# LepistaBioinformatics/classeq2

Hardware: AMD Instinct MI355X
Metric: query placements/sec, 10k-leaf tree, 150 bp reads (higher is better)
Workload: dtype u64

## Files before the change

### classeq2_amd/csrc/cls_api.cpp

```cpp
#include <hip/hip_runtime.h>
#include <ctype.h>
#include <stdio.h>
#include <stdlib.h>
#include <string.h>

#include <algorithm>
#include <mutex>
#include <new>
#include <string>
#include <thread>
#include <vector>

#include "cls_db.h"
#include "cls_device.h"
#include "cls_extract.h"
#include "cls_kernels.h"
#include "cls_pair.h"
#include "cls_place.h"
#include "cls_tally.h"
#include "cls_tuning.h"

namespace {

thread_local std::string g_err;
// ... 75 lines not shown
    uint64_t ws_seq = 0;
    std::vector<CallSlot> calls;
    struct TreeRow { uint64_t id; uint32_t pre, size; };
    std::vector<TreeRow> tree_rows;
};

namespace cls {
Tuning& tuning() {
    static Tuning t;
    return t;
}
}
namespace {
struct Knob { const char* name; int cls::Tuning::*field; };
const Knob KNOBS[] = {
    {"no_fast", &cls::Tuning::no_fast}, {"no_order", &cls::Tuning::no_order}, {"force_list", &cls::Tuning::force_list},
    {"no_mask_halves", &cls::Tuning::no_mask_halves}, {"no_fat_direct", &cls::Tuning::no_fat_direct}, {"no_tile", &cls::Tuning::no_tile}, {"tile_pass_codes", &cls::Tuning::tile_pass_codes}, {"tile_set_words", &cls::Tuning::tile_set_words}, {"time_class", &cls::Tuning::time_class}, {"tile_one_per_cu", &cls::Tuning::tile_one_per_cu}, {"tile_min_kmers", &cls::Tuning::tile_min_kmers}, {"no_tile_order", &cls::Tuning::no_tile_order}, {"tile_deal", &cls::Tuning::tile_deal}, {"blocks_per_cu", &cls::Tuning::blocks_per_cu}, {"key_blocks_per_cu", &cls::Tuning::key_blocks_per_cu},
    {"long_blocks_per_cu", &cls::Tuning::long_blocks_per_cu}, {"order_mode", &cls::Tuning::order_mode},
    {"order_windows", &cls::Tuning::order_windows}, {"order_both_strands", &cls::Tuning::order_both_strands},
    {"order_block_shift", &cls::Tuning::order_block_shift}, {"order_sample_shift", &cls::Tuning::order_sample_shift},
    {"profile_stop", &cls::Tuning::profile_stop}, {"timing", &cls::Tuning::timing},
    {"build_full_key", &cls::Tuning::build_full_key}, {"tally_no_wave_combine", &cls::Tuning::tally_no_wave_combine},
};
}

extern "C" int cls_set_tuning(const char* name, int value) {
    if (!name) return fail(CLS_E_INVALID_ARG, "cls_set_tuning: null name");
    for (const Knob& k : KNOBS)
        if (strcmp(k.name, name) == 0) { cls::tuning().*(k.field) = value; return CLS_OK; }
    return fail(CLS_E_INVALID_ARG, std::string("cls_set_tuning: unknown knob ") + name);
}
// ... 2078 lines not shown
```

### classeq2_amd/csrc/cls_device.h

```cpp
#pragma once
#include <stdint.h>

#include "cls_place.h"

namespace cls {

struct DNode {
    uint32_t pre;
    uint32_t size;
    uint32_t first_child;
    uint32_t n_nonleaf;
    uint64_t id;
    uint32_t split;
    uint32_t flags;
};
static_assert(sizeof(DNode) == 32, "DNode");

struct Slot {
    uint64_t hash;
    uint64_t loc;
};
static_assert(sizeof(Slot) == 16, "Slot");
constexpr uint64_t SLOT_EMPTY = ~0ULL;
struct TSlot {
// ... 58 lines not shown
    uint32_t max_nonleaf_arity;
    uint32_t format;
    uint32_t addr32;
    uint32_t binary_tree;
    uint32_t canonical;
    uint32_t set_bits;
    uint32_t n_sets;
};

struct PlaceParams {
    int32_t max_iterations;
    uint32_t remove_intersection;
    double min_match_coverage;
};

constexpr uint32_t MAX_READ_KMERS = 64 * 8 * 16;

}
```

### classeq2_amd/csrc/cls_kernels.h

```cpp
#pragma once
#include <hip/hip_runtime.h>

#include <string>
#include <tuple>
#include <type_traits>
#include <utility>

#include "cls_device.h"

namespace cls {

template <int V> using Int = std::integral_constant<int, V>;
template <class F> auto with_bool(bool b, F&& f) { return b ? f(std::true_type{}) : f(std::false_type{}); }
template <class... V> std::string instance_name(const char* kernel, V...) {
    auto arg = [](auto v) { if constexpr (std::is_same_v<decltype(v), bool>) return std::string(v ? "true" : "false"); else return std::to_string(v); };
    std::string s = std::string(kernel) + "<";
    const char* sep = "";
    ((s += sep + arg(V::value), sep = ", "), ...);
    return s + ">";
}
template <class F> struct Pick {
    F* fn;
    size_t smem;
    std::string name;
// ... 23 lines not shown
    uint32_t n_sub;
    TileCfg whole;
    uint64_t scratch_words;
    std::string name;
};

constexpr int N_LISTS = 8;

struct PlacePlan {
    uint32_t grid[2];
    uint32_t grid_blk;
    uint32_t grid_key;
    bool ordered;
    uint64_t keys_off_words;
    uint64_t sort_off_words;
    size_t sort_bytes;
    uint64_t child_off_words;
    uint32_t grid_long;
    uint32_t long_cap;
    uint32_t long_arity;
    uint64_t long_set;
    uint64_t long_stride_words;
    uint64_t long_off_words;
    uint32_t max_kmers;
    bool blk;
    bool tiled;
    TilePlan tile;
    uint32_t tile_from;
    uint64_t tile_off_words;
    enum Timed : uint8_t { TIME_CLASS0, TIME_BLOCK, TIME_TILE } timed;
// ... 18 lines not shown
```

### classeq2_amd/csrc/cls_kernels.hip

```cpp
#include <hip/hip_runtime.h>
#include <stdlib.h>

#include <algorithm>
#include <type_traits>

#include "cls_device.h"
#include "cls_devutil.h"
#include "cls_kernels.h"
#include "cls_murmur.h"
#include "cls_sort.h"
#include "cls_tuning.h"

namespace cls {

namespace {

constexpr int WAVES_PER_BLOCK = 4;
#ifndef MIN_WAVES_PER_EU
#define MIN_WAVES_PER_EU 4
#endif
#ifndef FAST_MIN_WAVES
#define FAST_MIN_WAVES 5
#endif
#ifndef CLS_NARROW_CANON_BITS
// ... 818 lines not shown
    for (int i = 0; i < 4; ++i) r.s[i] = p[i];
    return r;
}

struct FastCtx {
    uint8_t* ascii;
    uint32_t* packed;
    uint32_t* set;
    uint32_t* gkey;
    uint32_t* gcnt;
    uint4* stage;
    uint32_t* ccnt;
    uint32_t* conly;
    uint32_t* cpre;
};
constexpr int FAST_SLOTS_NARROW = 5;
constexpr uint32_t FAST_MAX_ARITY = 256;

struct FatRec { uint32_t x, vlo_lg, vhi_root; };
template <int SET_BITS>
__device__ __forceinline__ void clear_tables(const FastCtx& cx, uint32_t table_bits, uint32_t lane) {
    if constexpr (SET_BITS == 0) {
        if (lane == 0) cx.set[0] = SET_EMPTY;
    } else {
        const uint4 ones = make_uint4(SET_EMPTY, SET_EMPTY, SET_EMPTY, SET_EMPTY), zero = make_uint4(0, 0, 0, 0);
        uint4* const s4 = reinterpret_cast<uint4*>(cx.set);
        uint4* const k4 = reinterpret_cast<uint4*>(cx.gkey);
        uint4* const c4 = reinterpret_cast<uint4*>(cx.gcnt);
#pragma unroll 1
        for (uint32_t i = lane; i < (1u << table_bits) / 4; i += 64) { s4[i] = ones; k4[i] = ones; c4[i] = zero; }
    }
}

template <int SLOTS, int SET_BITS, bool ADDR32, bool FAT = false>
__device__ __forceinline__ bool fast_front(const DbDev& db, const FastCtx& cx, const uint8_t* __restrict__ bases, uint64_t b0,
                                           uint32_t L, uint32_t nf, uint32_t nk, uint32_t (&e)[SLOTS], uint32_t (&key)[SLOTS], uint32_t (&kw)[SLOTS],
                                           FatRec (&rec)[SLOTS], uint32_t sample_shift = 32, bool canonical = false, uint32_t table_bits = SET_BITS) {
    const uint32_t lane = threadIdx.x & 63;
    const uint32_t k = db.k;
    bool bad = false;
#pragma unroll 1
    for (uint32_t i = lane; i < L; i += 64) {
        uint8_t c = bases[b0 + i];
        if (c >= 'a' && c <= 'z') c -= 32;
        bad |= !(c == 'A' || c == 'C' || c == 'G' || c == 'T');
        cx.ascii[i] = c;
    }
    clear_tables<SET_BITS>(cx, table_bits, lane);
    if (__ballot(bad)) return false;
    wave_sync();
    {
        const uint32_t n_words = (L + 15) >> 4;
#pragma unroll 1
        for (uint32_t w = lane; w < n_words; w += 64) {
            uint32_t acc = 0;
#pragma unroll
            for (int q = 0; q < 4; ++q) {
                uint32_t t = *reinterpret_cast<const uint32_t*>(cx.ascii + 16 * w + 4 * q);
                t = (t >> 1) & 0x03030303u;
                t = (t | (t >> 6) | (t >> 12) | (t >> 18)) & 0xFFu;
                acc |= t << (8 * q);
            }
            cx.packed[w] = acc;
        }
    }
    wave_sync();
    const uint32_t* __restrict__ direct = db.direct;
    const uint32_t kmask = (k == 16) ? 0xFFFFFFFFu : ((1u << (2 * k)) - 1u);
#pragma unroll
    for (int s = 0; s < SLOTS; ++s) {
        const uint32_t j = s * 64 + lane;
        const bool valid = j < nk;
        const bool rc = j >= nf;
        const uint32_t p = valid ? (rc ? (nf - 1) - (j - nf) : j) : 0;
        const uint32_t w = p >> 4, sh = (2 * p) & 31;
        const uint32_t d0 = cx.packed[w], d1 = cx.packed[w + 1];
        uint32_t code = (uint32_t)((((uint64_t)d1 << 32) | d0) >> sh) & kmask;
        uint32_t rcc = __builtin_bitreverse32(code ^ (0xAAAAAAAAu & kmask));
        rcc = ((rcc >> 1) & 0x55555555u) | ((rcc & 0x55555555u) << 1);
        rcc >>= (32 - 2 * k);
        const bool palindrome = code == rcc;
        code = canonical ? (rcc < code ? rcc : code) : (rc ? rcc : code);
        const bool take = valid && (sample_shift >= 32 || ((code * 0x9E3779B1u) >> sample_shift) == 0);
        if constexpr (FAT) {
            const uint4 v = ldx<uint4, ADDR32>(reinterpret_cast<const uint4*>(db.direct16), take ? code : 0u);
            e[s] = take ? v.w : 0u;
            rec[s] = FatRec{v.x, take ? v.y : 0xFFFFFFFFu, take ? v.z : 0u};
        } else {
            const uint32_t v = ldx<uint32_t, ADDR32>(direct, take ? code : 0u);
            e[s] = take ? v : 0u;
        }
        key[s] = code;
        kw[s] = !take ? 0u : (canonical && !palindrome) ? 2u : 1u;
    }
    return true;
}

template <int SLOTS, int SET_BITS, bool ADDR32>
__device__ __forceinline__ bool hash_front(const DbDev& db, const FastCtx& cx, const uint8_t* __restrict__ bases, uint64_t b0,
                                           uint32_t L, uint32_t nf, uint32_t nk, uint32_t (&e)[SLOTS], uint32_t (&key)[SLOTS], uint32_t (&kw)[SLOTS],
                                           uint32_t table_bits, uint32_t& ib) {
    const uint32_t lane = threadIdx.x & 63;
    const uint32_t k = db.k, m_eff = db.m_eff;
    bool bad = false;
#pragma unroll 1
    for (uint32_t i = lane; i < L; i += 64) {
        uint8_t c = bases[b0 + i];
        if (c >= 'a' && c <= 'z') c -= 32;
        bad |= !(c == 'A' || c == 'C' || c == 'G' || c == 'T');
// ... 347 lines not shown
            for (uint32_t c = CL; c < n_loop; ++c) {
                uint4 g = cx.stage[c * 64 + lane];
                uint32_t sm, rm_, km;
                classify(g.x, g.y, g.w, sm, rm_, km);
                const uint2 t = request(g.z, rm_);
                finish(g.x, g.y, g.z, g.w, sm, rm_, km, t);
                cx.stage[c * 64 + lane] = g;
            }
        };
        if (right) narrow_side(std::true_type{}); else narrow_side(std::false_type{});
    }
}

template <int SLOTS, int SET_BITS, bool STATS, bool ADDR32, int MODE, bool POLY>
__device__ __forceinline__ void place_read_fast(const DbDev& db, const PlaceParams& prm, const FastCtx& cx,
                                                const uint8_t* __restrict__ bases, uint64_t b0, uint64_t b1, uint32_t r,
                                                cls_placement* __restrict__ out, cls_query_stats* __restrict__ stats,
                                                uint32_t profile_stop_arg) {
#ifdef CLS_PROFILE_HOOKS
    const uint32_t profile_stop = profile_stop_arg;
#else
    constexpr uint32_t profile_stop = 0;
    (void)profile_stop_arg;
#endif
    const uint32_t lane = threadIdx.x & 63;
    const uint32_t k = db.k;
    const uint64_t L64 = b1 - b0;
    auto put_stats = [&](uint32_t nk_, uint32_t nm, uint32_t nr, uint64_t lp) {
        if (STATS && stats && lane == 0) {
            uint64_t* s = reinterpret_cast<uint64_t*>(stats + r);
            s[0] = (uint64_t)nk_ | ((uint64_t)nm << 32);
            s[1] = (uint64_t)nr;
            s[2] = lp;
        }
    };
    if (L64 < k) { put_stats(0, 0, 0, 0); write_record(out, r, CLS_ERR_TOO_FEW_KMERS, 0, 0, 0, 0); return; }
    const uint32_t L = (uint32_t)L64, nf = L - k + 1, nk = 2 * nf;
    constexpr bool CANON = MODE == 1 || MODE == 4, HASHED = MODE == 2, FAT = MODE >= 3;
    constexpr int LS = CANON ? (SLOTS + 1) / 2 : SLOTS;
    uint32_t sid[LS], key[LS], kw[LS];
    FatRec frec[LS];
    uint32_t tb = SET_BITS;
    if constexpr (SET_BITS > 9) {
        const uint32_t want = 2 * (CANON ? nf : nk);
        tb = 9;
        while ((1u << tb) < want && tb < (uint32_t)SET_BITS) ++tb;
        tb = uniform(tb);
    }
    bool valid_read;
    uint32_t ib = 0;
    if constexpr (HASHED) valid_read = hash_front<LS, SET_BITS, ADDR32>(db, cx, bases, b0, L, nf, nk, sid, key, kw, tb, ib);
    else {
        valid_read = fast_front<LS, SET_BITS, ADDR32, FAT>(db, cx, bases, b0, L, nf, CANON ? nf : nk, sid, key, kw, frec, 32, CANON, tb);
        if (STATS) for (int s = 0; s < LS; ++s) ib += kw[s] ? (FAT ? 16u : 4u) : 0u;
    }
    auto put_index_bytes = [&]() {
        if constexpr (STATS) {
            const uint32_t total = wave_sum(ib);
            if (stats && lane == 0) reinterpret_cast<uint32_t*>(stats + r)[3] = total;
        }
    };
    if (!valid_read) {
        put_stats(0, 0, 0, 0);
        write_record(out, r, CLS_ERR_INVALID_BASE, 0, 0, 0, 0);
        return;
    }
    uint32_t nm_lane = 0;
#pragma unroll
    for (int s = 0; s < LS; ++s) {
        sid[s] &= SET_ID_MASK;
        if (sid[s] != 0) {
            uint32_t pos = (key[s] * 2654435761u) >> (32 - tb);
#pragma unroll 1
            for (;;) {
                const uint32_t old = atomicCAS(&cx.set[pos], SET_EMPTY, key[s]);
                if (old == SET_EMPTY) break;
                if (old == key[s]) { sid[s] = 0; kw[s] = 0; break; }
                pos = (pos + 1) & ((1u << tb) - 1);
            }
        }
        nm_lane += sid[s] != 0 ? kw[s] : 0u;
// ... 74 lines not shown
        const uint64_t exp_usize = (expected != expected) ? 0ull : (uint64_t)expected;
        if ((uint64_t)n_root < exp_usize) { put_index_bytes(); write_record(out, r, CLS_UNCLASSIFIABLE_COVERAGE, (int32_t)n_root, 0, 0, 0); return; }
    }
    bool in_registers = false;
    if constexpr (!POLY) in_registers = uniform(n_sets) <= 128;
    constexpr bool REG2 = !POLY || MODE != 2;
    if (in_registers) descend_groups<ADDR32, POLY, STATS, false, REG2>(db, prm, cx, n_sets, P, r, out, ib);
    else descend_groups<ADDR32, POLY, STATS, true, REG2>(db, prm, cx, n_sets, P, r, out, ib);
    put_index_bytes();
}

template <int SLOTS, int SET_BITS, bool STATS, bool ADDR32, int MODE, bool POLY>
__global__ __launch_bounds__(64 * WAVES_PER_BLOCK, SLOTS > 5 ? FAST_MIN_WAVES_WIDE : POLY ? FAST_MIN_WAVES_POLY : FAST_MIN_WAVES) void place_fast_kernel(
    DbDev db, PlaceParams prm, const uint8_t* __restrict__ bases, const uint64_t* __restrict__ offsets,
    const uint32_t* __restrict__ list, const uint32_t* __restrict__ list_len, uint32_t list_n, uint32_t xcd_chunks,
    cls_placement* __restrict__ out, cls_query_stats* __restrict__ stats, uint32_t ascii_cap, uint32_t profile_stop) {
    extern __shared__ __align__(16) uint8_t smem[];
    const uint32_t wave = threadIdx.x >> 6;
    const uint32_t packed_words = MODE == 2 ? 0u : ((ascii_cap >> 4) + 2 + 3) & ~3u;
    constexpr bool FITS = (12u << SET_BITS) >= 16u * 64 * ((MODE == 1 || MODE == 4) ? (SLOTS + 1) / 2 : SLOTS);
    if constexpr (FITS) {
    const uint32_t per_wave = ascii_cap + 4u * packed_words + (12u << SET_BITS) + (POLY ? 12u * FAST_MAX_ARITY + 16u : 0u);
    FastCtx cx;
    cx.ascii = smem + wave * per_wave;
    cx.packed = reinterpret_cast<uint32_t*>(cx.ascii + ascii_cap);
    cx.set = cx.packed + packed_words;
    cx.gkey = cx.set + (1u << SET_BITS);
    cx.gcnt = cx.gkey + (1u << SET_BITS);
    cx.stage = reinterpret_cast<uint4*>(cx.set);
    cx.ccnt = cx.gcnt + (1u << SET_BITS);
    cx.conly = cx.ccnt + FAST_MAX_ARITY;
    cx.cpre = cx.conly + FAST_MAX_ARITY;
    if (xcd_chunks && SLOTS > FAST_SLOTS_NARROW && *list_len == 0) return;
    const uint32_t n_list = xcd_chunks ? list_n : *list_len;
    const uint32_t xcd = blockIdx.x & 7u, bpx = gridDim.x >> 3;
    const uint32_t chunk = xcd_chunks ? (n_list + 7u) >> 3 : n_list;
    const uint32_t first = xcd_chunks ? (blockIdx.x >> 3) * WAVES_PER_BLOCK + wave : blockIdx.x * WAVES_PER_BLOCK + wave;
    const uint32_t stride = (xcd_chunks ? bpx : gridDim.x) * WAVES_PER_BLOCK;
    const uint32_t origin = xcd_chunks ? xcd * chunk : 0u;
    constexpr uint32_t cap = 64 * SLOTS;
    for (uint32_t ql = first; ql < chunk; ql += stride) {
        const uint32_t q = origin + ql;
        if (q >= n_list) break;
        const uint32_t r = list[q];
        const uint64_t b0 = offsets[r], b1 = offsets[r + 1];
        if (xcd_chunks) {
            const uint64_t L64 = b1 - b0;
            if (L64 >= db.k && 2 * (L64 - db.k + 1) > cap) continue;
            if (SLOTS > FAST_SLOTS_NARROW && (L64 < db.k || 2 * (L64 - db.k + 1) <= 64 * FAST_SLOTS_NARROW)) continue;
        }
        place_read_fast<SLOTS, SET_BITS, STATS, ADDR32, MODE, POLY>(db, prm, cx, bases, b0, b1, r, out, stats, profile_stop);
        wave_sync();
    }
    }
}

__device__ __forceinline__ uint64_t make_order_key(uint32_t key_mode, uint32_t median, uint32_t mh_spec, uint32_t mh_all, uint32_t block_shift, uint32_t set_bits) {
    if (key_mode == 1) return ((uint64_t)(mh_all >> 12) << set_bits) | median;
    return ((uint64_t)(median >> block_shift) << 16) | (mh_spec >> 16);
}

template <int SLOTS, bool ADDR32, bool FWD, bool HASHED>
__global__ __launch_bounds__(64 * WAVES_PER_BLOCK) void order_key_kernel(DbDev db, const uint8_t* __restrict__ bases,
                                                                       const uint64_t* __restrict__ offsets, uint32_t n_reads,
                                                                       uint64_t* __restrict__ keys, uint32_t* __restrict__ idx,
                                                                       uint32_t ascii_cap, uint32_t key_mode,
// ... 59 lines not shown
                    }
                    key = make_order_key(key_mode, prefix, mh, mha, block_shift, db.set_bits);
                }
            }
            wave_sync();
        }
        if (lane == 0) { keys[r] = key; idx[r] = r; }
    }
}

template <bool ADDR32>
__global__ __launch_bounds__(64 * WAVES_PER_BLOCK) void order_key_half_kernel(DbDev db, const uint8_t* __restrict__ bases,
                                                                            const uint64_t* __restrict__ offsets, uint32_t n_reads,
                                                                            uint64_t* __restrict__ keys, uint32_t* __restrict__ idx,
                                                                            uint32_t key_mode, uint32_t block_shift,
                                                                            uint32_t key_cap) {
    constexpr uint32_t MAXL = 64 + DIRECT_MAX_K - 1 + 1;
    constexpr uint32_t WORDS = (MAXL + 15) / 16 + 2;
    __shared__ __align__(16) uint8_t s_ascii[WAVES_PER_BLOCK * 2][(MAXL + 19) & ~3u];
    __shared__ uint32_t s_packed[WAVES_PER_BLOCK * 2][WORDS];
    const uint32_t wave = threadIdx.x >> 6, lane = threadIdx.x & 63, half = lane >> 5, hl = lane & 31;
    uint8_t* ascii = s_ascii[wave * 2 + half];
    uint32_t* packed = s_packed[wave * 2 + half];
    const uint32_t k = db.k;
    const uint32_t kmask = (1u << (2 * k)) - 1u;
    const uint32_t* __restrict__ direct = db.direct;
    const uint32_t pair0 = (blockIdx.x * WAVES_PER_BLOCK + wave) * 2, stride = gridDim.x * WAVES_PER_BLOCK * 2;
    auto half_of = [&](uint64_t m) { return (uint32_t)(m >> (32 * half)); };
    for (uint32_t r0 = pair0; r0 < n_reads; r0 += stride) {
        const uint32_t r = r0 + half;
        const bool have = r < n_reads;
        const uint64_t b0 = have ? offsets[r] : 0, L64 = have ? offsets[r + 1] - b0 : 0;
        const bool keyed = have && L64 >= k && 2 * (L64 - k + 1) <= (uint64_t)key_cap;
        const uint32_t L = keyed ? (uint32_t)std::min<uint64_t>(L64, 64 + k - 1) : 0, nf = keyed ? L - k + 1 : 0;
        bool bad = false;
        for (uint32_t i = hl; i < L; i += 32) {
            uint8_t c = bases[b0 + i];
            if (c >= 'a' && c <= 'z') c -= 32;
            bad |= !(c == 'A' || c == 'C' || c == 'G' || c == 'T');
            ascii[i] = c;
        }
        const bool ok = keyed && half_of(__ballot(bad)) == 0;
        wave_sync();
        for (uint32_t w = hl; w < (L + 15) / 16 + 1; w += 32) {
            uint32_t acc = 0;
#pragma unroll
            for (int q = 0; q < 4; ++q) {
                uint32_t t = *reinterpret_cast<const uint32_t*>(ascii + 16 * w + 4 * q);
                t = (t >> 1) & 0x03030303u;
                t = (t | (t >> 6) | (t >> 12) | (t >> 18)) & 0xFFu;
                acc |= t << (8 * q);
            }
            if (w < WORDS) packed[w] = acc;
        }
        wave_sync();
        uint32_t e[2], hs[2];
#pragma unroll
        for (int s = 0; s < 2; ++s) {
            const uint32_t p = hl + 32 * s;
            const bool valid = ok && p < nf;
            const uint32_t w = valid ? p >> 4 : 0, sh = valid ? (2 * p) & 31 : 0;
            const uint32_t d0 = packed[w], d1 = packed[w + 1];
            uint32_t code = (uint32_t)((((uint64_t)d1 << 32) | d0) >> sh) & kmask;
            uint32_t rcc = __builtin_bitreverse32(code ^ (0xAAAAAAAAu & kmask));
            rcc = ((rcc >> 1) & 0x55555555u) | ((rcc & 0x55555555u) << 1);
            rcc >>= (32 - 2 * k);
            code = rcc < code ? rcc : code;
            const uint32_t v = ldx<uint32_t, ADDR32>(direct, valid ? code : 0u);
            e[s] = valid ? v : 0u;
            hs[s] = mix32(code);
// ... 559 lines not shown
}
auto long_kernel(const DbDev& db, bool stats) {
    auto inst = [&](auto... v) { return pick(place_long_kernel<decltype(v)::value...>, 0, "place_long_kernel", v...); };
    return with_bool(db.format == FMT_SPLIT, [&](auto sp) { return with_bool(stats, [&](auto st) { return inst(sp, st); }); });
}

using KeyFn = decltype(order_key_kernel<2, true, true, false>);
using KeyHalfFn = decltype(order_key_half_kernel<true>);
struct KeyKernel {
    KeyFn* full;
    KeyHalfFn* half;
    size_t smem;
    std::string name;
    const void* fn() const { return full ? (const void*)full : (const void*)half; }
};
KeyKernel key_kernel(const DbDev& db, bool sizing) {
    const Tuning& tn = tuning();
    const bool fwd = !tn.order_both_strands, hashed = fast_mode(db) == 2;
    if (!sizing && !hashed && fwd && tn.order_windows == 64 && (uint32_t)tn.order_sample_shift >= 32)
        return with_bool(db.addr32, [&](auto a32) { return KeyKernel{nullptr, order_key_half_kernel<decltype(a32)::value>, 0, instance_name("order_key_half_kernel", a32)}; });
    const uint32_t ac = ascii_cap_of(db, 0);
    const size_t smem = (size_t)WAVES_PER_BLOCK * (ac + (db.direct ? 4u * (((ac >> 4) + 2 + 3) & ~3u) : 0u) + 16u);
    auto inst = [&](auto... v) { return KeyKernel{order_key_kernel<decltype(v)::value...>, nullptr, smem, instance_name("order_key_kernel", v...)}; };
    auto of = [&](auto a32, auto hs) {
        if (fwd && tn.order_windows <= 64) return inst(Int<2>{}, a32, std::true_type{}, hs);
        if (fwd || sizing) return inst(Int<CLS_SLOTS[0]>{}, a32, std::true_type{}, hs);
        return inst(Int<CLS_SLOTS[0]>{}, a32, std::false_type{}, hs);
    };
    if (hashed) return of(std::true_type{}, std::true_type{});
    return db.addr32 ? of(std::true_type{}, std::false_type{}) : of(std::false_type{}, std::false_type{});
}
}

void PlacePlan::class_caps(uint32_t (&cap)[N_LISTS]) const {
// ... 44 lines not shown
        p.grid[0] = std::max<uint32_t>(8, p.grid[0] & ~7u);
        p.grid[1] = std::max<uint32_t>(8, p.grid[1] & ~7u);
        {
            int per_cu = tuning().key_blocks_per_cu;
            const KeyKernel k = key_kernel(db, true);
            if (per_cu <= 0 && (hipOccupancyMaxActiveBlocksPerMultiprocessor(&per_cu, k.fn(), 64 * WAVES_PER_BLOCK, k.smem) != hipSuccess || per_cu <= 0)) per_cu = 4;
            if (tuning().key_blocks_per_cu <= 0 && fast_mode(db) == 2) per_cu *= 2;
            p.grid_key = std::max<uint32_t>(1, std::min<uint32_t>(want, n_cu * (uint32_t)per_cu));
        }
        p.keys_off_words = w;
        w += 6 * (uint64_t)n_reads;
        p.sort_off_words = w;
        p.sort_bytes = order_temp_bytes(n_reads);
        w += (p.sort_bytes + 3) / 4 + 2;
        w += w & 1;
    }
    p.child_off_words = w;
    w += child_words;
    w += w & 1;
    p.max_kmers = n_long ? std::max<uint32_t>(long_cap, 2u) : MAX_READ_KMERS;
    const uint32_t blk_cap = (uint32_t)(64 * BLK_WAVES * BLK_SLOTS);
    p.tile_from = blk_cap;
    if (tile_usable(db)) {
        p.tile_from = tuning().tile_min_kmers > 0 ? std::min<uint32_t>(blk_cap, (uint32_t)tuning().tile_min_kmers) : (uint32_t)(64 * CLS_SLOTS[1]);
        if (p.max_kmers > p.tile_from) {
            p.tile = tile_plan(db, stats, p.tile_from, p.max_kmers, n_reads, n_cu);
            p.tiled = p.tile.whole.cap_kmers > p.tile_from;
        }
    }
    if (p.tiled) {
// ... 32 lines not shown
    for (int c = 0; c < N_LISTS; ++c) lists[c] = d_ws + 16 + (size_t)c * n_reads;
    uint32_t* child_ws = (child_ws_stride(db) && !child_in_lds(db)) ? d_ws + plan.child_off_words : nullptr;
    hipError_t e = hipMemsetAsync(counts, 0, 64, stream);
    if (e != hipSuccess) return e;
    const uint32_t profile_stop = (uint32_t)tuning().profile_stop;
    const uint32_t ws_stride = child_ws_stride(db);
    const bool st = d_stats != nullptr;
    auto classify = [&](const uint32_t* order) {
        ClassCaps caps{};
        plan.class_caps(caps.cap);
        return launch_kernel(classify_kernel, dim3((n_reads + CLASSIFY_THREADS * CLASSIFY_PER_THREAD - 1) / (CLASSIFY_THREADS * CLASSIFY_PER_THREAD)), dim3(CLASSIFY_THREADS), 0,
                             stream, d_offsets, order, n_reads, db.k, caps, lists[0], counts, d_out, d_stats);
    };
    const uint32_t* list0 = lists[0];
    uint32_t list0_n = 0, xcd_chunks = 0;
    if (!plan.ordered) e = classify(nullptr);
    else {
        uint64_t* keys_in = reinterpret_cast<uint64_t*>(d_ws + plan.keys_off_words);
        uint64_t* keys_out = keys_in + n_reads;
        uint32_t* idx_in = reinterpret_cast<uint32_t*>(keys_out + n_reads);
        uint32_t* idx_out = idx_in + n_reads;
        const Tuning& tn = tuning();
        const uint32_t key_mode = (uint32_t)tn.order_mode;
        const uint32_t block_shift = (uint32_t)tn.order_block_shift;
        const uint32_t key_cap = (plan.tiled && !tn.no_tile_order) ? 0xFFFFFFFFu : (uint32_t)(64 * CLS_SLOTS[1]);
        const KeyKernel k = key_kernel(db, false);
        const dim3 block(64 * WAVES_PER_BLOCK);
        if (k.half) {
            const uint32_t grid_half = std::max<uint32_t>(1, std::min<uint32_t>((n_reads + 2 * WAVES_PER_BLOCK - 1) / (2 * WAVES_PER_BLOCK), plan.grid_key));
            e = launch_kernel(k.half, dim3(grid_half), block, k.smem, stream, db, d_bases, d_offsets, n_reads, keys_in, idx_in, key_mode, block_shift, key_cap);
        } else {
            e = launch_kernel(k.full, dim3(plan.grid_key), block, k.smem, stream, db, d_bases, d_offsets, n_reads, keys_in, idx_in, ascii_cap_of(db, 0), key_mode,
                              block_shift, (uint32_t)tn.order_sample_shift, tn.order_both_strands ? 0u : 1u, key_cap);
        }
        if (e != hipSuccess) return e;
        e = order_reads(d_ws + plan.sort_off_words, keys_in, idx_out, n_reads, order_key_bits(db) - 1, stream);
        if (e != hipSuccess) return e;
        list0 = idx_out;
        list0_n = n_reads;
        xcd_chunks = 1;
        e = classify(idx_out);
    }
    if (e != hipSuccess) return e;
    auto launch_class = [&](int c) {
        const ClassKernel k = class_kernel(db, c, st);
        const dim3 grid(plan.grid[c]), block(64 * WAVES_PER_BLOCK);
        if (k.fast) {
            return launch_kernel(k.fast, grid, block, k.smem, stream, db, prm, d_bases, d_offsets, xcd_chunks ? list0 : lists[c], counts + c, list0_n, xcd_chunks,
                                 d_out, d_stats, ascii_cap_of(db, c), profile_stop);
        }
        if (k.split)
            return launch_kernel(k.split, grid, block, k.smem, stream, db, prm, d_bases, d_offsets, lists[c], counts + c, d_out, d_stats, seq_cap_of(db, c),
                                 profile_stop, child_ws, ws_stride);
        return launch_kernel(k.wave, grid, block, k.smem, stream, db, prm, d_bases, d_offsets, lists[c], counts + c, d_out, d_stats, seq_cap_of(db, c), child_ws,
                             ws_stride);
    };
    auto timed = [&](PlacePlan::Timed t, auto&& launch) {
        if (ev_start && plan.timed == t) (void)hipEventRecord(ev_start, stream);
        const hipError_t r = launch();
        if (ev_stop && plan.timed == t) (void)hipEventRecord(ev_stop, stream);
        return r;
    };
    e = timed(PlacePlan::TIME_CLASS0, [&] { return launch_class(0); });
    if (e != hipSuccess) return e;
// ... 31 lines not shown
```

### classeq2_amd/csrc/cls_sort.h

```cpp
#pragma once
#include <hip/hip_runtime.h>
#include <stddef.h>
#include <stdint.h>

namespace cls {
constexpr int ORDER_BIN_BITS = 12;
constexpr uint32_t ORDER_BINS = 1u << ORDER_BIN_BITS;
size_t order_temp_bytes(uint32_t n);
hipError_t order_reads(void* tmp, const uint64_t* keys, uint32_t* idx_out, uint32_t n, int key_bits, hipStream_t stream);
}
```

### classeq2_amd/csrc/cls_sort.hip

```cpp
#include "cls_sort.h"

namespace cls {

namespace {

constexpr int SORT_THREADS = 1024, SORT_PER_THREAD = 16;

__device__ __forceinline__ uint32_t bin_of(uint64_t key, int shift) {
    return key == ~0ull ? ORDER_BINS - 1 : (uint32_t)(key >> shift) & (ORDER_BINS - 1);
}

__global__ __launch_bounds__(SORT_THREADS) void order_hist_kernel(const uint64_t* __restrict__ keys, uint32_t n, int shift, uint32_t* __restrict__ hist,
                                                                 uint32_t* __restrict__ block_base) {
    __shared__ uint32_t h[ORDER_BINS];
    for (uint32_t i = threadIdx.x; i < ORDER_BINS; i += SORT_THREADS) h[i] = 0;
    __syncthreads();
    const uint32_t base = blockIdx.x * (SORT_THREADS * SORT_PER_THREAD);
#pragma unroll
    for (int q = 0; q < SORT_PER_THREAD; ++q) {
        const uint32_t r = base + q * SORT_THREADS + threadIdx.x;
        if (r < n) atomicAdd(&h[bin_of(keys[r], shift)], 1u);
    }
    __syncthreads();
    for (uint32_t i = threadIdx.x; i < ORDER_BINS; i += SORT_THREADS)
// ... 8 lines not shown
    for (uint32_t q = 0; q < PER; ++q) { v[q] = hist[threadIdx.x * PER + q]; sum += v[q]; }
    const uint32_t lane = threadIdx.x & 63, wave = threadIdx.x >> 6;
    uint32_t inc = sum;
#pragma unroll
    for (int o = 1; o < 64; o <<= 1) { const uint32_t t = __shfl_up(inc, o); if ((int)lane >= o) inc += t; }
    if (lane == 63) wave_tot[wave] = inc;
    __syncthreads();
    uint32_t before = 0;
    for (uint32_t w = 0; w < wave; ++w) before += wave_tot[w];
    uint32_t at = before + inc - sum;
#pragma unroll
    for (uint32_t q = 0; q < PER; ++q) { hist[threadIdx.x * PER + q] = at; at += v[q]; }
}

__global__ __launch_bounds__(SORT_THREADS) void order_scatter_kernel(const uint64_t* __restrict__ keys, uint32_t n, int shift, const uint32_t* __restrict__ start,
                                                                    const uint32_t* __restrict__ block_base, uint32_t* __restrict__ idx_out) {
    __shared__ uint32_t at[ORDER_BINS];
    for (uint32_t i = threadIdx.x; i < ORDER_BINS; i += SORT_THREADS) at[i] = start[i] + block_base[(size_t)blockIdx.x * ORDER_BINS + i];
    __syncthreads();
    const uint32_t base = blockIdx.x * (SORT_THREADS * SORT_PER_THREAD);
#pragma unroll
    for (int q = 0; q < SORT_PER_THREAD; ++q) {
        const uint32_t r = base + q * SORT_THREADS + threadIdx.x;
        if (r < n) idx_out[atomicAdd(&at[bin_of(keys[r], shift)], 1u)] = r;
    }
}

}

static uint32_t order_blocks(uint32_t n) { return (n + SORT_THREADS * SORT_PER_THREAD - 1) / (SORT_THREADS * SORT_PER_THREAD); }

size_t order_temp_bytes(uint32_t n) { return (1 + (size_t)order_blocks(n)) * ORDER_BINS * sizeof(uint32_t); }

hipError_t order_reads(void* tmp, const uint64_t* keys, uint32_t* idx_out, uint32_t n, int key_bits, hipStream_t stream) {
    uint32_t* hist = static_cast<uint32_t*>(tmp);
    uint32_t* block_base = hist + ORDER_BINS;
    const int shift = key_bits > ORDER_BIN_BITS ? key_bits - ORDER_BIN_BITS : 0;
    hipError_t e = hipMemsetAsync(hist, 0, ORDER_BINS * sizeof(uint32_t), stream);
    if (e != hipSuccess) return e;
    const uint32_t blocks = order_blocks(n);
    hipLaunchKernelGGL(order_hist_kernel, dim3(blocks), dim3(SORT_THREADS), 0, stream, keys, n, shift, hist, block_base);
    hipLaunchKernelGGL(order_scan_kernel, dim3(1), dim3(1024), 0, stream, hist);
    hipLaunchKernelGGL(order_scatter_kernel, dim3(blocks), dim3(SORT_THREADS), 0, stream, keys, n, shift, (const uint32_t*)hist, (const uint32_t*)block_base, idx_out);
    return hipGetLastError();
}

}
```

### classeq2_amd/csrc/cls_tuning.h

```cpp
#pragma once

namespace cls {

struct Tuning {
    int no_fast = 0;
    int no_order = 0;
    int force_list = 0;
    int no_mask_halves = 0;
    int no_fat_direct = 0;
    int no_tile = 0;
    int tile_pass_codes = 0;
    int tile_set_words = 0;
    int tile_min_kmers = 0;
    int tile_deal = 64;
    int no_tile_order = 0;
    int tile_one_per_cu = 0;
    int time_class = 0;
    int blocks_per_cu = 0;
    int key_blocks_per_cu = 0;
    int long_blocks_per_cu = 2;
    int order_mode = 0;
    int order_windows = 64;
    int order_both_strands = 0;
    int order_block_shift = 2;
// ... 11 lines not shown
```

Measured before the change: 158.0 million.

## Pack narrow reads into 2-bit records in key kernel and scatter them sorted

The order-key kernel, which already reads and validates every base, now also writes a fixed 64-byte record per read holding the read id, length/status header and 2-bit packed bases. The sort scatter step permutes these records into sorted order alongside the index. The narrow fast placement kernel then loads one contiguous record per read instead of gathering ASCII bases through offsets and re-packing them. This removes scattered base gathers and the per-read packing stage from the placement kernel, at the cost of extra workspace and record traffic in the key and scatter kernels.

```diff
diff --git a/classeq2_amd/csrc/cls_api.cpp b/classeq2_amd/csrc/cls_api.cpp
--- a/classeq2_amd/csrc/cls_api.cpp
+++ b/classeq2_amd/csrc/cls_api.cpp
@@ -113,7 +113,7 @@
 namespace {
 struct Knob { const char* name; int cls::Tuning::*field; };
 const Knob KNOBS[] = {
-    {"no_fast", &cls::Tuning::no_fast}, {"no_order", &cls::Tuning::no_order}, {"force_list", &cls::Tuning::force_list},
+    {"no_fast", &cls::Tuning::no_fast}, {"no_order", &cls::Tuning::no_order}, {"no_packed_reads", &cls::Tuning::no_packed_reads}, {"force_list", &cls::Tuning::force_list},
     {"no_mask_halves", &cls::Tuning::no_mask_halves}, {"no_fat_direct", &cls::Tuning::no_fat_direct}, {"no_tile", &cls::Tuning::no_tile}, {"tile_pass_codes", &cls::Tuning::tile_pass_codes}, {"tile_set_words", &cls::Tuning::tile_set_words}, {"time_class", &cls::Tuning::time_class}, {"tile_one_per_cu", &cls::Tuning::tile_one_per_cu}, {"tile_min_kmers", &cls::Tuning::tile_min_kmers}, {"no_tile_order", &cls::Tuning::no_tile_order}, {"tile_deal", &cls::Tuning::tile_deal}, {"blocks_per_cu", &cls::Tuning::blocks_per_cu}, {"key_blocks_per_cu", &cls::Tuning::key_blocks_per_cu},
     {"long_blocks_per_cu", &cls::Tuning::long_blocks_per_cu}, {"order_mode", &cls::Tuning::order_mode},
     {"order_windows", &cls::Tuning::order_windows}, {"order_both_strands", &cls::Tuning::order_both_strands},
diff --git a/classeq2_amd/csrc/cls_device.h b/classeq2_amd/csrc/cls_device.h
--- a/classeq2_amd/csrc/cls_device.h
+++ b/classeq2_amd/csrc/cls_device.h
@@ -96,6 +96,12 @@
     double min_match_coverage;
 };
 
+constexpr uint32_t PACKED_READ_DWORDS = 16, PACKED_READ_WORDS = 12, PACKED_READ_MAX_BASES = 176;
+constexpr uint32_t PACKED_READ_LEN_MASK = 0xFFFFu;
+constexpr uint32_t PACKED_READ_PACKED = 1u << 16;
+constexpr uint32_t PACKED_READ_BAD_BASE = 1u << 17;
+constexpr uint32_t PACKED_READ_OTHER_CLASS = 1u << 18;
+
 constexpr uint32_t MAX_READ_KMERS = 64 * 8 * 16;
 
 }
diff --git a/classeq2_amd/csrc/cls_kernels.h b/classeq2_amd/csrc/cls_kernels.h
--- a/classeq2_amd/csrc/cls_kernels.h
+++ b/classeq2_amd/csrc/cls_kernels.h
@@ -61,6 +61,9 @@
     bool ordered;
     uint64_t keys_off_words;
     uint64_t sort_off_words;
+    bool packed;
+    uint64_t rec_in_off_words;
+    uint64_t rec_sorted_off_words;
     size_t sort_bytes;
     uint64_t child_off_words;
     uint32_t grid_long;
diff --git a/classeq2_amd/csrc/cls_kernels.hip b/classeq2_amd/csrc/cls_kernels.hip
--- a/classeq2_amd/csrc/cls_kernels.hip
+++ b/classeq2_amd/csrc/cls_kernels.hip
@@ -856,6 +856,7 @@
     uint32_t* conly;
     uint32_t* cpre;
 };
+constexpr uint32_t REC_PRESENT = 1u << 31;
 constexpr int FAST_SLOTS_NARROW = 5;
 constexpr uint32_t FAST_MAX_ARITY = 256;
 
@@ -874,12 +875,9 @@
     }
 }
 
-template <int SLOTS, int SET_BITS, bool ADDR32, bool FAT = false>
-__device__ __forceinline__ bool fast_front(const DbDev& db, const FastCtx& cx, const uint8_t* __restrict__ bases, uint64_t b0,
-                                           uint32_t L, uint32_t nf, uint32_t nk, uint32_t (&e)[SLOTS], uint32_t (&key)[SLOTS], uint32_t (&kw)[SLOTS],
-                                           FatRec (&rec)[SLOTS], uint32_t sample_shift = 32, bool canonical = false, uint32_t table_bits = SET_BITS) {
+template <int SET_BITS>
+__device__ __forceinline__ bool fast_stage(const FastCtx& cx, const uint8_t* __restrict__ bases, uint64_t b0, uint32_t L, uint32_t table_bits) {
     const uint32_t lane = threadIdx.x & 63;
-    const uint32_t k = db.k;
     bool bad = false;
 #pragma unroll 1
     for (uint32_t i = lane; i < L; i += 64) {
@@ -906,7 +904,14 @@
             cx.packed[w] = acc;
         }
     }
-    wave_sync();
+    return true;
+}
+
+template <int SLOTS, bool ADDR32, bool FAT>
+__device__ __forceinline__ void fast_lookup(const DbDev& db, const FastCtx& cx, uint32_t nf, uint32_t nk, uint32_t (&e)[SLOTS], uint32_t (&key)[SLOTS],
+                                            uint32_t (&kw)[SLOTS], FatRec (&rec)[SLOTS], uint32_t sample_shift, bool canonical) {
+    const uint32_t lane = threadIdx.x & 63;
+    const uint32_t k = db.k;
     const uint32_t* __restrict__ direct = db.direct;
     const uint32_t kmask = (k == 16) ? 0xFFFFFFFFu : ((1u << (2 * k)) - 1u);
 #pragma unroll
@@ -935,6 +940,15 @@
         key[s] = code;
         kw[s] = !take ? 0u : (canonical && !palindrome) ? 2u : 1u;
     }
+}
+
+template <int SLOTS, int SET_BITS, bool ADDR32, bool FAT = false>
+__device__ __forceinline__ bool fast_front(const DbDev& db, const FastCtx& cx, const uint8_t* __restrict__ bases, uint64_t b0,
+                                           uint32_t L, uint32_t nf, uint32_t nk, uint32_t (&e)[SLOTS], uint32_t (&key)[SLOTS], uint32_t (&kw)[SLOTS],
+                                           FatRec (&rec)[SLOTS], uint32_t sample_shift = 32, bool canonical = false, uint32_t table_bits = SET_BITS) {
+    if (!fast_stage<SET_BITS>(cx, bases, b0, L, table_bits)) return false;
+    wave_sync();
+    fast_lookup<SLOTS, ADDR32, FAT>(db, cx, nf, nk, e, key, kw, rec, sample_shift, canonical);
     return true;
 }
 
@@ -1312,9 +1326,9 @@
 
 template <int SLOTS, int SET_BITS, bool STATS, bool ADDR32, int MODE, bool POLY>
 __device__ __forceinline__ void place_read_fast(const DbDev& db, const PlaceParams& prm, const FastCtx& cx,
-                                                const uint8_t* __restrict__ bases, uint64_t b0, uint64_t b1, uint32_t r,
+                                                const uint8_t* __restrict__ bases, uint64_t b0, uint32_t L, uint32_t r,
                                                 cls_placement* __restrict__ out, cls_query_stats* __restrict__ stats,
-                                                uint32_t profile_stop_arg) {
+                                                uint32_t profile_stop_arg, uint32_t rec_hdr) {
 #ifdef CLS_PROFILE_HOOKS
     const uint32_t profile_stop = profile_stop_arg;
 #else
@@ -1323,7 +1337,6 @@
 #endif
     const uint32_t lane = threadIdx.x & 63;
     const uint32_t k = db.k;
-    const uint64_t L64 = b1 - b0;
     auto put_stats = [&](uint32_t nk_, uint32_t nm, uint32_t nr, uint64_t lp) {
         if (STATS && stats && lane == 0) {
             uint64_t* s = reinterpret_cast<uint64_t*>(stats + r);
@@ -1332,8 +1345,8 @@
             s[2] = lp;
         }
     };
-    if (L64 < k) { put_stats(0, 0, 0, 0); write_record(out, r, CLS_ERR_TOO_FEW_KMERS, 0, 0, 0, 0); return; }
-    const uint32_t L = (uint32_t)L64, nf = L - k + 1, nk = 2 * nf;
+    if (L < k) { put_stats(0, 0, 0, 0); write_record(out, r, CLS_ERR_TOO_FEW_KMERS, 0, 0, 0, 0); return; }
+    const uint32_t nf = L - k + 1, nk = 2 * nf;
     constexpr bool CANON = MODE == 1 || MODE == 4, HASHED = MODE == 2, FAT = MODE >= 3;
     constexpr int LS = CANON ? (SLOTS + 1) / 2 : SLOTS;
     uint32_t sid[LS], key[LS], kw[LS];
@@ -1345,11 +1358,21 @@
         while ((1u << tb) < want && tb < (uint32_t)SET_BITS) ++tb;
         tb = uniform(tb);
     }
+    uint32_t ib = 0;
     bool valid_read;
-    uint32_t ib = 0;
     if constexpr (HASHED) valid_read = hash_front<LS, SET_BITS, ADDR32>(db, cx, bases, b0, L, nf, nk, sid, key, kw, tb, ib);
-    else {
-        valid_read = fast_front<LS, SET_BITS, ADDR32, FAT>(db, cx, bases, b0, L, nf, CANON ? nf : nk, sid, key, kw, frec, 32, CANON, tb);
+    else if (rec_hdr) {
+        valid_read = (rec_hdr & PACKED_READ_PACKED) != 0;
+        if (valid_read) clear_tables<SET_BITS>(cx, tb, lane);
+    } else valid_read = fast_stage<SET_BITS>(cx, bases, b0, L, tb);
+    if (!valid_read) {
+        put_stats(0, 0, 0, 0);
+        write_record(out, r, CLS_ERR_INVALID_BASE, 0, 0, 0, 0);
+        return;
+    }
+    if constexpr (!HASHED) {
+        wave_sync();
+        fast_lookup<LS, ADDR32, FAT>(db, cx, nf, CANON ? nf : nk, sid, key, kw, frec, 32, CANON);
         if (STATS) for (int s = 0; s < LS; ++s) ib += kw[s] ? (FAT ? 16u : 4u) : 0u;
     }
     auto put_index_bytes = [&]() {
@@ -1358,11 +1381,6 @@
             if (stats && lane == 0) reinterpret_cast<uint32_t*>(stats + r)[3] = total;
         }
     };
-    if (!valid_read) {
-        put_stats(0, 0, 0, 0);
-        write_record(out, r, CLS_ERR_INVALID_BASE, 0, 0, 0, 0);
-        return;
-    }
     uint32_t nm_lane = 0;
 #pragma unroll
     for (int s = 0; s < LS; ++s) {
@@ -1467,7 +1485,8 @@
 __global__ __launch_bounds__(64 * WAVES_PER_BLOCK, SLOTS > 5 ? FAST_MIN_WAVES_WIDE : POLY ? FAST_MIN_WAVES_POLY : FAST_MIN_WAVES) void place_fast_kernel(
     DbDev db, PlaceParams prm, const uint8_t* __restrict__ bases, const uint64_t* __restrict__ offsets,
     const uint32_t* __restrict__ list, const uint32_t* __restrict__ list_len, uint32_t list_n, uint32_t xcd_chunks,
-    cls_placement* __restrict__ out, cls_query_stats* __restrict__ stats, uint32_t ascii_cap, uint32_t profile_stop) {
+    cls_placement* __restrict__ out, cls_query_stats* __restrict__ stats, uint32_t ascii_cap, uint32_t profile_stop,
+    const uint32_t* __restrict__ recs) {
     extern __shared__ __align__(16) uint8_t smem[];
     const uint32_t wave = threadIdx.x >> 6;
     const uint32_t packed_words = MODE == 2 ? 0u : ((ascii_cap >> 4) + 2 + 3) & ~3u;
@@ -1495,14 +1514,29 @@
     for (uint32_t ql = first; ql < chunk; ql += stride) {
         const uint32_t q = origin + ql;
         if (q >= n_list) break;
-        const uint32_t r = list[q];
-        const uint64_t b0 = offsets[r], b1 = offsets[r + 1];
-        if (xcd_chunks) {
-            const uint64_t L64 = b1 - b0;
-            if (L64 >= db.k && 2 * (L64 - db.k + 1) > cap) continue;
-            if (SLOTS > FAST_SLOTS_NARROW && (L64 < db.k || 2 * (L64 - db.k + 1) <= 64 * FAST_SLOTS_NARROW)) continue;
-        }
-        place_read_fast<SLOTS, SET_BITS, STATS, ADDR32, MODE, POLY>(db, prm, cx, bases, b0, b1, r, out, stats, profile_stop);
+        uint32_t r, L, rec_hdr = 0;
+        uint64_t b0 = 0;
+        if (SLOTS == FAST_SLOTS_NARROW && MODE != 2 && xcd_chunks && recs) {
+            uint32_t lane = threadIdx.x & 63;
+            asm volatile("" : "+v"(lane));
+            const uint32_t w = lane < PACKED_READ_DWORDS ? recs[(size_t)q * PACKED_READ_DWORDS + lane] : 0u;
+            r = (uint32_t)__builtin_amdgcn_readlane((int)w, 0);
+            rec_hdr = (uint32_t)__builtin_amdgcn_readlane((int)w, 1);
+            if (rec_hdr & PACKED_READ_OTHER_CLASS) continue;
+            if (lane >= 2 && lane < 2 + PACKED_READ_WORDS) cx.packed[lane - 2] = w;
+            L = rec_hdr & PACKED_READ_LEN_MASK;
+            rec_hdr |= REC_PRESENT;
+        } else {
+            r = list[q];
+            b0 = offsets[r];
+            const uint64_t L64 = offsets[r + 1] - b0;
+            if (xcd_chunks) {
+                if (L64 >= db.k && 2 * (L64 - db.k + 1) > cap) continue;
+                if (SLOTS > FAST_SLOTS_NARROW && (L64 < db.k || 2 * (L64 - db.k + 1) <= 64 * FAST_SLOTS_NARROW)) continue;
+            }
+            L = (uint32_t)L64;
+        }
+        place_read_fast<SLOTS, SET_BITS, STATS, ADDR32, MODE, POLY>(db, prm, cx, bases, b0, L, r, out, stats, profile_stop, rec_hdr);
         wave_sync();
     }
     }
@@ -1592,16 +1626,18 @@
                                                                             const uint64_t* __restrict__ offsets, uint32_t n_reads,
                                                                             uint64_t* __restrict__ keys, uint32_t* __restrict__ idx,
                                                                             uint32_t key_mode, uint32_t block_shift,
-                                                                            uint32_t key_cap) {
-    constexpr uint32_t MAXL = 64 + DIRECT_MAX_K - 1 + 1;
-    constexpr uint32_t WORDS = (MAXL + 15) / 16 + 2;
-    __shared__ __align__(16) uint8_t s_ascii[WAVES_PER_BLOCK * 2][(MAXL + 19) & ~3u];
+                                                                            uint32_t key_cap, uint32_t* __restrict__ recs) {
+    constexpr uint32_t MAXL = PACKED_READ_MAX_BASES;
+    constexpr uint32_t WORDS = MAXL / 16 + 2;
+    static_assert(MAXL % 16 == 0 && MAXL >= 64 * FAST_SLOTS_NARROW / 2 + DIRECT_MAX_K - 1 && MAXL / 16 + 1 <= PACKED_READ_WORDS, "packed-read record");
+    __shared__ __align__(16) uint8_t s_ascii[WAVES_PER_BLOCK * 2][MAXL + 16];
     __shared__ uint32_t s_packed[WAVES_PER_BLOCK * 2][WORDS];
     const uint32_t wave = threadIdx.x >> 6, lane = threadIdx.x & 63, half = lane >> 5, hl = lane & 31;
     uint8_t* ascii = s_ascii[wave * 2 + half];
     uint32_t* packed = s_packed[wave * 2 + half];
     const uint32_t k = db.k;
     const uint32_t kmask = (1u << (2 * k)) - 1u;
+    const uint32_t key_len = 64 + k - 1;
     const uint32_t* __restrict__ direct = db.direct;
     const uint32_t pair0 = (blockIdx.x * WAVES_PER_BLOCK + wave) * 2, stride = gridDim.x * WAVES_PER_BLOCK * 2;
     auto half_of = [&](uint64_t m) { return (uint32_t)(m >> (32 * half)); };
@@ -1610,15 +1646,20 @@
         const bool have = r < n_reads;
         const uint64_t b0 = have ? offsets[r] : 0, L64 = have ? offsets[r + 1] - b0 : 0;
         const bool keyed = have && L64 >= k && 2 * (L64 - k + 1) <= (uint64_t)key_cap;
-        const uint32_t L = keyed ? (uint32_t)std::min<uint64_t>(L64, 64 + k - 1) : 0, nf = keyed ? L - k + 1 : 0;
-        bool bad = false;
+        const bool narrow = recs && have && L64 >= k && 2 * (L64 - k + 1) <= (uint64_t)(64 * FAST_SLOTS_NARROW);
+        const uint32_t L = narrow ? (uint32_t)L64 : keyed ? (uint32_t)std::min<uint64_t>(L64, key_len) : 0;
+        const uint32_t nf = keyed ? std::min<uint32_t>(L, key_len) - k + 1 : 0;
+        bool bad = false, bad_key = false;
         for (uint32_t i = hl; i < L; i += 32) {
             uint8_t c = bases[b0 + i];
             if (c >= 'a' && c <= 'z') c -= 32;
-            bad |= !(c == 'A' || c == 'C' || c == 'G' || c == 'T');
+            const bool b = !(c == 'A' || c == 'C' || c == 'G' || c == 'T');
+            bad |= b;
+            bad_key |= b && i < key_len;
             ascii[i] = c;
         }
-        const bool ok = keyed && half_of(__ballot(bad)) == 0;
+        const bool ok = keyed && half_of(__ballot(bad_key)) == 0;
+        const bool all_ok = half_of(__ballot(bad)) == 0;
         wave_sync();
         for (uint32_t w = hl; w < (L + 15) / 16 + 1; w += 32) {
             uint32_t acc = 0;
@@ -1629,9 +1670,18 @@
                 t = (t | (t >> 6) | (t >> 12) | (t >> 18)) & 0xFFu;
                 acc |= t << (8 * q);
             }
+            const uint32_t in = 16 * w >= L ? 0u : L - 16 * w;
+            if (in < 16) acc &= (1u << (2 * in)) - 1u;
             if (w < WORDS) packed[w] = acc;
         }
         wave_sync();
+        if (recs && have && hl < PACKED_READ_DWORDS) {
+            const bool too_long = L64 >= k && !narrow;
+            const uint32_t hdr = too_long ? PACKED_READ_OTHER_CLASS
+                                          : (uint32_t)L64 | (!narrow ? 0u : all_ok ? PACKED_READ_PACKED : PACKED_READ_BAD_BASE);
+            const bool words = narrow && all_ok && hl >= 2 && hl < 2 + PACKED_READ_WORDS && hl - 2 < (L + 15) / 16 + 1;
+            recs[(size_t)r * PACKED_READ_DWORDS + hl] = hl == 0 ? r : hl == 1 ? hdr : words ? packed[hl - 2] : 0u;
+        }
         uint32_t e[2], hs[2];
 #pragma unroll
         for (int s = 0; s < 2; ++s) {
@@ -2221,10 +2271,15 @@
     std::string name;
     const void* fn() const { return full ? (const void*)full : (const void*)half; }
 };
+bool key_is_half(const DbDev& db) {
+    const Tuning& tn = tuning();
+    return fast_mode(db) != 2 && !tn.order_both_strands && tn.order_windows == 64 && (uint32_t)tn.order_sample_shift >= 32;
+}
+bool use_packed_reads(const DbDev& db, uint32_t n_reads) { return use_order(db, n_reads) && key_is_half(db) && !tuning().no_packed_reads; }
 KeyKernel key_kernel(const DbDev& db, bool sizing) {
     const Tuning& tn = tuning();
     const bool fwd = !tn.order_both_strands, hashed = fast_mode(db) == 2;
-    if (!sizing && !hashed && fwd && tn.order_windows == 64 && (uint32_t)tn.order_sample_shift >= 32)
+    if (!sizing && key_is_half(db))
         return with_bool(db.addr32, [&](auto a32) { return KeyKernel{nullptr, order_key_half_kernel<decltype(a32)::value>, 0, instance_name("order_key_half_kernel", a32)}; });
     const uint32_t ac = ascii_cap_of(db, 0);
     const size_t smem = (size_t)WAVES_PER_BLOCK * (ac + (db.direct ? 4u * (((ac >> 4) + 2 + 3) & ~3u) : 0u) + 16u);
@@ -2299,6 +2354,14 @@
         p.sort_bytes = order_temp_bytes(n_reads);
         w += (p.sort_bytes + 3) / 4 + 2;
         w += w & 1;
+        p.packed = use_packed_reads(db, n_reads);
+        if (p.packed) {
+            w = (w + 15) & ~15ull;
+            p.rec_in_off_words = w;
+            w += (uint64_t)PACKED_READ_DWORDS * n_reads;
+            p.rec_sorted_off_words = w;
+            w += (uint64_t)PACKED_READ_DWORDS * n_reads;
+        }
     }
     p.child_off_words = w;
     w += child_words;
@@ -2361,6 +2424,7 @@
     };
     const uint32_t* list0 = lists[0];
     uint32_t list0_n = 0, xcd_chunks = 0;
+    uint32_t* recs = nullptr;
     if (!plan.ordered) e = classify(nullptr);
     else {
         uint64_t* keys_in = reinterpret_cast<uint64_t*>(d_ws + plan.keys_off_words);
@@ -2373,15 +2437,18 @@
         const uint32_t key_cap = (plan.tiled && !tn.no_tile_order) ? 0xFFFFFFFFu : (uint32_t)(64 * CLS_SLOTS[1]);
         const KeyKernel k = key_kernel(db, false);
         const dim3 block(64 * WAVES_PER_BLOCK);
+        uint32_t* rec_in = plan.packed && k.half ? d_ws + plan.rec_in_off_words : nullptr;
+        if (rec_in) recs = d_ws + plan.rec_sorted_off_words;
         if (k.half) {
             const uint32_t grid_half = std::max<uint32_t>(1, std::min<uint32_t>((n_reads + 2 * WAVES_PER_BLOCK - 1) / (2 * WAVES_PER_BLOCK), plan.grid_key));
-            e = launch_kernel(k.half, dim3(grid_half), block, k.smem, stream, db, d_bases, d_offsets, n_reads, keys_in, idx_in, key_mode, block_shift, key_cap);
+            e = launch_kernel(k.half, dim3(grid_half), block, k.smem, stream, db, d_bases, d_offsets, n_reads, keys_in, idx_in, key_mode, block_shift, key_cap,
+                              rec_in);
         } else {
             e = launch_kernel(k.full, dim3(plan.grid_key), block, k.smem, stream, db, d_bases, d_offsets, n_reads, keys_in, idx_in, ascii_cap_of(db, 0), key_mode,
                               block_shift, (uint32_t)tn.order_sample_shift, tn.order_both_strands ? 0u : 1u, key_cap);
         }
         if (e != hipSuccess) return e;
-        e = order_reads(d_ws + plan.sort_off_words, keys_in, idx_out, n_reads, order_key_bits(db) - 1, stream);
+        e = order_reads(d_ws + plan.sort_off_words, keys_in, idx_out, n_reads, order_key_bits(db) - 1, stream, rec_in, recs);
         if (e != hipSuccess) return e;
         list0 = idx_out;
         list0_n = n_reads;
@@ -2394,7 +2461,7 @@
         const dim3 grid(plan.grid[c]), block(64 * WAVES_PER_BLOCK);
         if (k.fast) {
             return launch_kernel(k.fast, grid, block, k.smem, stream, db, prm, d_bases, d_offsets, xcd_chunks ? list0 : lists[c], counts + c, list0_n, xcd_chunks,
-                                 d_out, d_stats, ascii_cap_of(db, c), profile_stop);
+                                 d_out, d_stats, ascii_cap_of(db, c), profile_stop, c == 0 ? recs : nullptr);
         }
         if (k.split)
             return launch_kernel(k.split, grid, block, k.smem, stream, db, prm, d_bases, d_offsets, lists[c], counts + c, d_out, d_stats, seq_cap_of(db, c),
diff --git a/classeq2_amd/csrc/cls_sort.h b/classeq2_amd/csrc/cls_sort.h
--- a/classeq2_amd/csrc/cls_sort.h
+++ b/classeq2_amd/csrc/cls_sort.h
@@ -7,5 +7,6 @@
 constexpr int ORDER_BIN_BITS = 12;
 constexpr uint32_t ORDER_BINS = 1u << ORDER_BIN_BITS;
 size_t order_temp_bytes(uint32_t n);
-hipError_t order_reads(void* tmp, const uint64_t* keys, uint32_t* idx_out, uint32_t n, int key_bits, hipStream_t stream);
+hipError_t order_reads(void* tmp, const uint64_t* keys, uint32_t* idx_out, uint32_t n, int key_bits, hipStream_t stream, const void* rec_in = nullptr,
+                       void* rec_out = nullptr);
 }
diff --git a/classeq2_amd/csrc/cls_sort.hip b/classeq2_amd/csrc/cls_sort.hip
--- a/classeq2_amd/csrc/cls_sort.hip
+++ b/classeq2_amd/csrc/cls_sort.hip
@@ -46,7 +46,8 @@
 }
 
 __global__ __launch_bounds__(SORT_THREADS) void order_scatter_kernel(const uint64_t* __restrict__ keys, uint32_t n, int shift, const uint32_t* __restrict__ start,
-                                                                    const uint32_t* __restrict__ block_base, uint32_t* __restrict__ idx_out) {
+                                                                    const uint32_t* __restrict__ block_base, uint32_t* __restrict__ idx_out,
+                                                                    const uint4* __restrict__ rec_in, uint4* __restrict__ rec_out) {
     __shared__ uint32_t at[ORDER_BINS];
     for (uint32_t i = threadIdx.x; i < ORDER_BINS; i += SORT_THREADS) at[i] = start[i] + block_base[(size_t)blockIdx.x * ORDER_BINS + i];
     __syncthreads();
@@ -54,7 +55,16 @@
 #pragma unroll
     for (int q = 0; q < SORT_PER_THREAD; ++q) {
         const uint32_t r = base + q * SORT_THREADS + threadIdx.x;
-        if (r < n) idx_out[atomicAdd(&at[bin_of(keys[r], shift)], 1u)] = r;
+        if (r < n) {
+            const uint32_t pos = atomicAdd(&at[bin_of(keys[r], shift)], 1u);
+            idx_out[pos] = r;
+            if (rec_in) {
+                const uint4* src = rec_in + 4 * (size_t)r;
+                uint4* dst = rec_out + 4 * (size_t)pos;
+                const uint4 a = src[0], b = src[1], c = src[2], d = src[3];
+                dst[0] = a; dst[1] = b; dst[2] = c; dst[3] = d;
+            }
+        }
     }
 }
 
@@ -64,7 +74,7 @@
 
 size_t order_temp_bytes(uint32_t n) { return (1 + (size_t)order_blocks(n)) * ORDER_BINS * sizeof(uint32_t); }
 
-hipError_t order_reads(void* tmp, const uint64_t* keys, uint32_t* idx_out, uint32_t n, int key_bits, hipStream_t stream) {
+hipError_t order_reads(void* tmp, const uint64_t* keys, uint32_t* idx_out, uint32_t n, int key_bits, hipStream_t stream, const void* rec_in, void* rec_out) {
     uint32_t* hist = static_cast<uint32_t*>(tmp);
     uint32_t* block_base = hist + ORDER_BINS;
     const int shift = key_bits > ORDER_BIN_BITS ? key_bits - ORDER_BIN_BITS : 0;
@@ -73,7 +83,8 @@
     const uint32_t blocks = order_blocks(n);
     hipLaunchKernelGGL(order_hist_kernel, dim3(blocks), dim3(SORT_THREADS), 0, stream, keys, n, shift, hist, block_base);
     hipLaunchKernelGGL(order_scan_kernel, dim3(1), dim3(1024), 0, stream, hist);
-    hipLaunchKernelGGL(order_scatter_kernel, dim3(blocks), dim3(SORT_THREADS), 0, stream, keys, n, shift, (const uint32_t*)hist, (const uint32_t*)block_base, idx_out);
+    hipLaunchKernelGGL(order_scatter_kernel, dim3(blocks), dim3(SORT_THREADS), 0, stream, keys, n, shift, (const uint32_t*)hist, (const uint32_t*)block_base, idx_out,
+                       static_cast<const uint4*>(rec_in), static_cast<uint4*>(rec_out));
     return hipGetLastError();
 }
 
diff --git a/classeq2_amd/csrc/cls_tuning.h b/classeq2_amd/csrc/cls_tuning.h
--- a/classeq2_amd/csrc/cls_tuning.h
+++ b/classeq2_amd/csrc/cls_tuning.h
@@ -5,6 +5,7 @@
 struct Tuning {
     int no_fast = 0;
     int no_order = 0;
+    int no_packed_reads = 0;
     int force_list = 0;
     int no_mask_halves = 0;
     int no_fat_direct = 0;
```

After: 158.7 million, median of 6. No clear change (+0.4%).
